# joe5saia/Hmc.jl

Measured on AMD Instinct MI355X. Metric: Gibbs draws/sec (whole node), 3-state T=1000 x256 windows per GPU, higher is better.
Workload: dtype f64

## Files before the change

hmc.jl_amd/csrc/gibbs_device.hpp:

```cpp
#pragma once
#include <hip/hip_runtime.h>
#include <stdint.h>

#include "../../include/hmcg.h"
#include "round5.hpp"

namespace hmcg {

enum { SITE_SIG2 = 0, SITE_MU = 1, SITE_RHO = 2, SITE_A = 3, SITE_X = 4, SITE_NOISE = 5 };
constexpr int GAMMA_MAX_ATTEMPTS = 64;
constexpr double INVSQRT2PI = 0.3989422804014327;
constexpr double TWO_PI = 6.283185307179586476925286766559;
constexpr double EPS64 = 2.220446049250313e-16;

struct KernelParams {
    const double* Y;
    const int32_t* T;
    const double* yreal;
    int32_t ldY, W, H;
    int32_t sweep_begin;
    int32_t sweep_end;
    int32_t resume;
    int32_t final_launch;
    int32_t horizons[HMCG_MAXH];
// ... 491 lines not shown
#pragma unroll
    for (int s = 0; s < K; ++s) {
        const uint32_t bs = (b >> (4 * s)) & 15u;
        m |= ((a >> (4u * bs)) & 15u) << (4 * s);
    }
    return m;
}
__device__ __forceinline__ int map_apply(uint32_t m, int s) { return (int)((m >> (4 * s)) & 15u); }

constexpr uint32_t BMAP_IDENTITY = 0x03020100u;
__device__ __forceinline__ uint32_t bmap_const(int v) { return (uint32_t)v * 0x01010101u; }
__device__ __forceinline__ uint32_t bmap_compose(uint32_t a, uint32_t b) { return __builtin_amdgcn_perm(a, a, b); }
__device__ __forceinline__ int bmap_apply(uint32_t m, int s) { return (int)((m >> (8 * s)) & 0xFFu); }
constexpr int DPP_ROW_SHL1 = 0x101, DPP_ROW_SHL2 = 0x102, DPP_ROW_SHL4 = 0x104, DPP_ROW_SHL8 = 0x108, DPP_WAVE_SHL1 = 0x130;

template <int K>
__device__ inline void matmul_small(double (&out)[K][K], const double (&a)[K][K], const double (&b)[K][K])
{
    double t[K][K];
#pragma unroll
    for (int i = 0; i < K; ++i)
#pragma unroll
        for (int j = 0; j < K; ++j) {
            double acc = 0.0;
#pragma unroll
            for (int k = 0; k < K; ++k) acc += a[i][k] * b[k][j];
            t[i][j] = acc;
        }
#pragma unroll
    for (int i = 0; i < K; ++i)
#pragma unroll
        for (int j = 0; j < K; ++j) out[i][j] = t[i][j];
}

template <int K>
__device__ inline double forecast_value(const double (&mu)[K], const double (&A)[K][K], const double (&pe)[K], int h)
{
    double M[K][K], v[K];
#pragma unroll
    for (int i = 0; i < K; ++i) {
        v[i] = mu[i];
#pragma unroll
        for (int j = 0; j < K; ++j) M[i][j] = A[i][j];
    }
    for (unsigned hh = (unsigned)h; hh != 0; hh >>= 1) {
        if (hh & 1u) {
            double nv[K];
#pragma unroll
            for (int i = 0; i < K; ++i) {
                double acc = 0.0;
#pragma unroll
                for (int j = 0; j < K; ++j) acc = fma(M[i][j], v[j], acc);
                nv[i] = acc;
            }
#pragma unroll
            for (int i = 0; i < K; ++i) v[i] = nv[i];
        }
        if (hh > 1u) matmul_small<K>(M, M, M);
    }
    double f = 0.0;
#pragma unroll
    for (int i = 0; i < K; ++i) f = fma(pe[i], v[i], f);
    return f;
}


template <int K>
struct ThetaBuf {
    double mu[K], sig2[K], isd[K], coef[K], rho[K];
    double A[K][K];
    double pi_end[K];
};

template <int K>
struct RngBuf {
    static constexpr int NG = K + K * K;
    double x[NG][2];
    double lu[NG][2];
    double uu[NG][2];
    double z[K];
    double rho[K];
};

template <int K, int L, int NT, bool SIG>
struct SweepShared {
    static constexpr int NW = NT / 64;
    static constexpr int NCNT = K + K * K;
    static constexpr int NF = K * K + (SIG ? K : 0);
    static constexpr int FW = (64 * L < 1024) ? 10 : 16;
    static constexpr int FPK = 32 / FW;
    static constexpr int NPK = (NF + FPK - 1) / FPK;
    unsigned red_pk[NW][NPK];
    double red_s1[SIG ? NW : 1][K];
    double red_s2[SIG ? NW : 1][K];
    int x_end;
    double red_d1[NW][K];
    double red_d2[NW][K];
    double pivot[K];
    ThetaBuf<K> th[2];
    RngBuf<K> rb[2];
    double wtot[NW][K * K];
    double pfirst[NT + 1][K];
    uint32_t wmap[NW];
    double ulast;
    int xfirst[NT + 1];
    double bred[NW];
    int selcnt[2][8][3];
    double ux[NT * L];
    double exptab[EXPTAB_N * EXPTAB_C];
    struct OutConst { double* base; double yr; int packed; int h; };
    OutConst oc[2][64];
    double ftail[2][SIG ? HMCG_MAXTAIL : 1][K];
    double pf_rep[2][K];
    double y_last[2];
};

template <int NW>
__device__ __forceinline__ double block_sum(double v, double* bred, int wave, int lane)
{
    v = wave_sum(v);
    __syncthreads();
    if (lane == 0 && wave < NW) bred[wave] = v;
    __syncthreads();
    double t = 0.0;
#pragma unroll
    for (int w = 0; w < NW; ++w) t += bred[w];
    return t;
}
template <int NW>
__device__ __forceinline__ double block_minmax(double v, double* bred, int wave, int lane, bool is_max)
{
    v = is_max ? wave_max(v) : wave_min(v);
    __syncthreads();
    if (lane == 0 && wave < NW) bred[wave] = v;
    __syncthreads();
    double t = bred[0];
#pragma unroll
    for (int w = 1; w < NW; ++w) t = is_max ? fmax(t, bred[w]) : fmin(t, bred[w]);
    return t;
}

__device__ __forceinline__ unsigned long long order_key(double v)
{
    const long long b = __double_as_longlong(v + 0.0);
    return (unsigned long long)(b ^ ((b >> 63) | (long long)0x8000000000000000ull));
}
__device__ __forceinline__ double key_value(unsigned long long k)
{
    return __longlong_as_double((long long)((k >> 63) ? (k ^ 0x8000000000000000ull) : ~k));
}
template <int NW, int NE, typename ElemFn>
__device__ __forceinline__ unsigned long long block_select(int n, ElemFn elem, int r, int (*cnt)[8][3], int wave, int lane)
{
    unsigned long long prefix = 0ull, mask = 0ull;
    const bool mine = __builtin_amdgcn_readfirstlane(wave) < NW;
    for (int b = 62; b >= 0; b -= 2) {
        const int par = (b >> 1) & 1;
        if (mine) {
            int c0 = 0, c1 = 0, c2 = 0;
            auto one = [&](int i) __attribute__((always_inline)) {
                unsigned long long key;
                const bool live = elem(i, key);
                const bool cand = live && ((key ^ prefix) & mask) == 0ull;
                const unsigned digit = (unsigned)(key >> b) & 3u;
                c0 += __builtin_popcountll(__builtin_amdgcn_ballot_w64(cand && digit == 0u));
                c1 += __builtin_popcountll(__builtin_amdgcn_ballot_w64(cand && digit == 1u));
                c2 += __builtin_popcountll(__builtin_amdgcn_ballot_w64(cand && digit == 2u));
            };
            if constexpr (NE > 0) {
#pragma unroll
                for (int i = 0; i < NE; ++i) one(i);
            } else {
                for (int i = 0; i < n; ++i) one(i);
            }
            if (lane == 0) { cnt[par][wave][0] = c0; cnt[par][wave][1] = c1; cnt[par][wave][2] = c2; }
        }
        __syncthreads();
        int t0 = 0, t1 = 0, t2 = 0;
#pragma unroll
        for (int w = 0; w < NW; ++w) { t0 += cnt[par][w][0]; t1 += cnt[par][w][1]; t2 += cnt[par][w][2]; }
        t0 = __builtin_amdgcn_readfirstlane(t0); t1 = __builtin_amdgcn_readfirstlane(t1); t2 = __builtin_amdgcn_readfirstlane(t2);
        unsigned long long digit = 0ull;
        if (r >= t0) { r -= t0; digit = 1ull;
            if (r >= t1) { r -= t1; digit = 2ull;
                if (r >= t2) { r -= t2; digit = 3ull; } } }
        prefix |= digit << b;
        mask |= 3ull << b;
    }
    return prefix;
}

template <int K>
__device__ __forceinline__ void sort_order(const double (&mu)[K], int (&order)[K])
{
    int pos[K];
#pragma unroll
    for (int i = 0; i < K; ++i) {
        int c = 0;
#pragma unroll
        for (int j = 0; j < K; ++j) c += (mu[j] < mu[i] || (mu[j] == mu[i] && j < i)) ? 1 : 0;
        pos[i] = c;
    }
#pragma unroll
    for (int q = 0; q < K; ++q) {
        int o = 0;
#pragma unroll
        for (int i = 0; i < K; ++i) o += (pos[i] == q) ? i : 0;
        order[q] = o;
    }
}

#ifdef HMCG_STAMPS
#define HMCG_NSTAMP 20
#define HMCG_NSTAMP_ALL (HMCG_NSTAMP + 2)
#define STAMP(i)                                                          \
    do {                                                                  \
        __builtin_amdgcn_sched_barrier(0);                                \
        asm volatile("; HMCG_STAMP_MARK %0" :: "n"(i));                    \
        const unsigned long long t_ = __builtin_amdgcn_s_memtime();       \
        __builtin_amdgcn_s_waitcnt(0xC07F);                               \
        __builtin_amdgcn_sched_barrier(0);                                \
        stamp_acc[i] += t_ - stamp_prev;                                  \
        stamp_prev = t_;                                                  \
    } while (0)
#else
#define STAMP(i)
#endif


template <int K, int L, int NT, bool SIG = false, bool SMOOTH = false, int NH = 0, int OCC = 1>
__global__ __launch_bounds__(NT + 64 * NH) __attribute__((amdgpu_waves_per_eu(OCC)))
void gibbs_sweeps_kernel(const KernelParams p)
{
    static_assert(NH == 0 || (NH == 4 && NT == 256), "helper waves: 256 + 256 threads");
    static_assert(K >= 2 && K <= 4, "small-K kernel: byte-per-entry state maps (v_perm_b32 composition)");
    static_assert(NT % 64 == 0 && NT >= 128, "at least two whole waves (wave 0 draws, the others work in its shadow)");
    constexpr int NW = NT / 64;
    constexpr int KK = K * K;
    constexpr int NG = K + KK;
    static_assert(NG <= 64, "draw roles must fit wave 0");
    using Sh = SweepShared<K, L, NT, SIG>;
    __shared__ Sh sh;

    int w_ = blockIdx.x;
    int t_lo_ = INT32_MIN, t_hi_ = INT32_MAX;
    if (p.order) {
        const int n_live = p.order[0];
        t_lo_ = p.order[1]; t_hi_ = p.order[2];
        if (n_live >= 0) {
            if (w_ >= n_live) __builtin_amdgcn_endpgm();
            w_ = p.order[4 + w_];
        }
    }
    const int w = w_;
#ifdef HMCG_VECTOR_WAVE
    const int tid = threadIdx.x, lane = tid & 63, wave = tid >> 6;
#else
    const int tid = threadIdx.x, lane = tid & 63, wave = __builtin_amdgcn_readfirstlane(tid >> 6);
#endif
    const int T = p.T[w];
    const int t0 = tid * L;
    const int owner = (T - 1) / L, l_last = (T - 1) % L;
    const bool helper = NH > 0 && __builtin_amdgcn_readfirstlane(wave) >= NW;
    int st = 0;

    if (T <= t_lo_ || T > t_hi_) __builtin_amdgcn_endpgm();
    if (T < 2 || T > NT * L || T > p.ldY) {
        if (tid == 0) flag_skipped(p, w, HMCG_ST_BAD_T);
        return;
    }

    exptab_fill(sh.exptab, tid, NT + 64 * NH);
    constexpr int XPAD = K < 4 ? K : 0;
    constexpr bool PADMARK = K < 4;
    double y[L];
    int x[L];
    bool bad = false;
#pragma unroll
    for (int l = 0; l < L; ++l) {
        const bool v = (t0 + l) < T;
        y[l] = v ? p.Y[(size_t)w * p.ldY + t0 + l] : 0.0;
        bad |= v && !isfinite(y[l]);
        x[l] = XPAD;
    }
    if (__syncthreads_or(bad ? 1 : 0)) {
        if (tid == 0) flag_skipped(p, w, HMCG_ST_NONFINITE);
        return;
    }
    int sb = T, se = T;
    double yreal[SIG ? L : 1];
    const double kfac = SIG ? 1.0 / (1.0 + p.kappa) : 1.0;
    if constexpr (SIG) {
        if (p.sig_range) { sb = p.sig_range[2 * w]; se = p.sig_range[2 * w + 1]; }
        bool bad_range = sb < 0 || se > T || (sb < se && se != T);
        if (p.save_range) {
            const int svb = p.save_range[2 * w], sve = p.save_range[2 * w + 1];
            bad_range |= svb < 0 || sve > T || (svb < sve && p.sigvals && sve - svb > p.nsave_ld);
        }
        if (bad_range) {
            if (tid == 0) flag_skipped(p, w, HMCG_ST_BAD_RANGE);
            return;
        }
        if (sb >= se) { sb = T; se = T; }
#pragma unroll
        for (int l = 0; l < L; ++l) yreal[l] = y[l];
    }
    int tail = 0;
    if constexpr (SIG) {
        if (p.end_pos) tail = (T - 1) - p.end_pos[w];
        if (tail < 0 || tail > HMCG_MAXTAIL || tail > T - 1) {
            if (tid == 0) flag_skipped(p, w, HMCG_ST_BAD_T);
            return;
        }
    }
    (void)kfac; (void)yreal; (void)sb; (void)se; (void)tail;

    double part = 0.0;
#pragma unroll
    for (int l = 0; l < L; ++l) part += y[l];
    const double xi = block_sum<NW>(part, sh.bred, wave, lane) / (double)T;

    double pivot[K];
#pragma unroll
    for (int k = 0; k < K; ++k) pivot[k] = xi;
// ... 234 lines not shown
            } else {
                double mu_u[K], pe_u[K], A_u[K][K];
#pragma unroll
                for (int i = 0; i < K; ++i) {
                    mu_u[i] = th.mu[i]; pe_u[i] = th.pi_end[i];
#pragma unroll
                    for (int j = 0; j < K; ++j) A_u[i][j] = th.A[i][j];
                }
                fv = forecast_value<K>(mu_u, A_u, pe_u, fc_h);
            }
            val = (o_which == 5) ? fv - fc_yr : fv;
        } else {
            double mu_u[K];
            int order[K];
#pragma unroll
            for (int i = 0; i < K; ++i) mu_u[i] = th.mu[i];
            sort_order<K>(mu_u, order);
            int si = 0, sj = 0;
#pragma unroll
            for (int qq = 0; qq < K; ++qq) {
                si = (qq == (o_which == 3 ? o_i : o_q)) ? order[qq] : si;
                sj = (qq == o_j) ? order[qq] : sj;
            }
            const double* src = o_which == 0 ? &th.mu[0] : (o_which == 1 ? &th.sig2[0] : (o_which == 2 ? &th.pi_end[0] : &th.A[0][0]));
            val = src[o_which == 3 ? si * K + sj : si];
            if constexpr (SIG) {
                if (tail > 0 && o_which == 2) {
                    double b[K];
#pragma unroll
                    for (int r = 0; r < K; ++r) b[r] = 1.0;
                    for (int j = tail - 1; j >= 0; --j) {
                        double g[K], nb[K];
#pragma unroll
                        for (int c = 0; c < K; ++c) g[c] = sh.ftail[sw & 1][j][c] * b[c];
#pragma unroll
                        for (int r = 0; r < K; ++r) {
                            double acc = 0.0;
#pragma unroll
                            for (int c = 0; c < K; ++c) acc = fma(th.A[r][c], g[c], acc);
                            nb[r] = acc;
                        }
                        rescale_pow2<K>(nb);
#pragma unroll
                        for (int r = 0; r < K; ++r) b[r] = nb[r];
                    }
                    double tot = 0.0, mine = 0.0;
#pragma unroll
                    for (int c = 0; c < K; ++c) {
                        const double g = sh.pf_rep[sw & 1][c] * b[c];
                        tot += g;
                        mine = (c == si) ? g : mine;
                    }
                    val = mine / tot;
                }
            }
        }
        if (out_base) ((__attribute__((address_space(1))) double*)out_base)[d - p.draw_off] = val;
        const double r5 = round5(val);
        sum_acc += r5;
        if constexpr (SIG) {
            if (p.sample_summary) {
                smp_acc += r5;
                const int smp = sw / p.per_sample;
                if (sw + 1 == (smp + 1) * p.per_sample) {
                    const int orole = (c.packed >> 20) & 63;
                    p.sample_summary[((size_t)w * p.n_samples + smp) * NS + orole] = p.nrun_s > 0 ? smp_acc / (double)p.nrun_s : __builtin_nan("");
                    smp_acc = 0.0;
                }
            }
        }
    };

#ifdef HMCG_STAMPS
    unsigned long long stamp_acc[HMCG_NSTAMP];
    unsigned long long stamp_prev = 0;
#endif
    constexpr int PB = L <= 1 ? 1 : (L <= 3 ? 2 : (L <= 7 ? 3 : (L <= 15 ? 4 : 5)));
    constexpr int FPW = 32 / PB;
    constexpr int NF = Sh::NF;
    constexpr int NWORD = (NF + FPW - 1) / FPW;
    constexpr int NPK = Sh::NPK;
    constexpr bool PADCNT = PADMARK && !SIG && NWORD == 1 && NF < FPW;
    static_assert(64 * L < 65536, "wave totals fit their fields (10 bits while 64 L < 1024, else 16)");
    auto publish_stats = [&]() __attribute__((always_inline)) {
        unsigned acc[NWORD];
#pragma unroll
        for (int wd = 0; wd < NWORD; ++wd) acc[wd] = 0;
#pragma unroll
        for (int l = 0; l < L; ++l) {
            const int xn = (l + 1 < L) ? x[(l + 1 < L) ? l + 1 : l] : xnext;
            const int code = PADCNT ? x[l] + K * xn : x[l] * K + xn;
            const bool pv = (t0 + l + 1) < T;
            if constexpr (PADCNT) {
                acc[0] += 1u << (PB * min(code, KK));
            } else if constexpr (NWORD == 1) {
                acc[0] += pv ? (1u << (PB * code)) : 0u;
            } else {
#pragma unroll
                for (int wd = 0; wd < NWORD; ++wd) {
                    const int rel = code - wd * FPW;
                    acc[wd] += (pv && rel >= 0 && rel < FPW) ? (1u << (PB * rel)) : 0u;
                }
            }
            if constexpr (SIG) {
                const int t = t0 + l;
                const bool sv = t >= sb && t < se;
                const int c2 = KK + x[l];
#pragma unroll
                for (int wd = 0; wd < NWORD; ++wd) {
                    const int rel = c2 - wd * FPW;
                    acc[wd] += (sv && rel >= 0 && rel < FPW) ? (1u << (PB * rel)) : 0u;
                }
            }
        }
        unsigned pk[NPK];
#pragma unroll
        for (int d = 0; d < NPK; ++d) {
            unsigned v = 0;
#pragma unroll
            for (int q = 0; q < Sh::FPK; ++q) {
                const int e = Sh::FPK * d + q;
                if (e < NF) v |= ((acc[e / FPW] >> (PB * (e % FPW))) & ((1u << PB) - 1u)) << (Sh::FW * q);
            }
            pk[d] = v;
        }
        wave_sum_words_lane63<NPK>(pk);
        double d1[K], d2[K], s1[SIG ? K : 1], s2[SIG ? K : 1];
#pragma unroll
        for (int i = 0; i < K; ++i) { d1[i] = 0.0; d2[i] = 0.0; }
        if constexpr (SIG) {
#pragma unroll
            for (int i = 0; i < K; ++i) { s1[i] = 0.0; s2[i] = 0.0; }
        }
#pragma unroll
        for (int l = 0; l < L; ++l) {
            double pvt = pivot[0];
#pragma unroll
            for (int k = 1; k < K; ++k) pvt = (x[l] == k) ? pivot[k] : pvt;
            const double dl = y[l] - pvt;
            const int t = t0 + l;
            const bool issig = SIG && t >= sb && t < se;
            const int xs = PADMARK ? (issig ? -1 : x[l]) : ((t < T && !issig) ? x[l] : -1);
#pragma unroll
            for (int i = 0; i < K; ++i) {
                const double dm = (xs == i) ? dl : 0.0;
                d1[i] += dm;
                d2[i] = fma(dm, dm, d2[i]);
            }
            if constexpr (SIG) {
                const int xg = issig ? x[l] : -1;
#pragma unroll
                for (int i = 0; i < K; ++i) {
                    const double dm = (xg == i) ? dl : 0.0;
                    s1[i] += dm;
                    s2[i] = fma(dm, dm, s2[i]);
                }
            }
        }
        if constexpr (SIG) {
            static_assert(!SIG || K <= 4, "signal path: transposed reduce carries 2 x 4 slots");
            double v8[8], o0, o1;
#pragma unroll
            for (int i = 0; i < 4; ++i) { v8[i] = i < K ? s1[i < K ? i : 0] : 0.0; v8[4 + i] = i < K ? s2[i < K ? i : 0] : 0.0; }
            wave_sum8_transposed(v8, lane, o0, o1);
            if ((lane & 0x3C) == 12) {
                const int i0 = lane & 2, i1 = i0 + 1;
                double* dst = (lane & 1) ? &sh.red_s2[wave][0] : &sh.red_s1[wave][0];
                if (i0 < K) dst[i0] = o0;
                if (i1 < K) dst[i1] = o1;
            }
        }
        if constexpr (K <= 4) {
            double v8[8], o0, o1;
#pragma unroll
            for (int i = 0; i < 4; ++i) { v8[i] = i < K ? d1[i] : 0.0; v8[4 + i] = i < K ? d2[i] : 0.0; }
            wave_sum8_transposed(v8, lane, o0, o1);
            if ((lane & 0x3C) == 12) {
                const int i0 = lane & 2, i1 = i0 + 1;
                double* dst = (lane & 1) ? &sh.red_d2[wave][0] : &sh.red_d1[wave][0];
                if (i0 < K) dst[i0] = o0;
                if (i1 < K) dst[i1] = o1;
            }
        } else {
#pragma unroll
            for (int i = 0; i < K; ++i) { d1[i] = wave_sum(d1[i]); d2[i] = wave_sum(d2[i]); }
            if (lane == 0) {
#pragma unroll
                for (int i = 0; i < K; ++i) { sh.red_d1[wave][i] = d1[i]; sh.red_d2[wave][i] = d2[i]; }
            }
        }
        if (lane == 63) {
#pragma unroll
            for (int d = 0; d < NPK; ++d) sh.red_pk[wave][d] = pk[d];
        }
        if (tid == 0) {
#pragma unroll
            for (int k = 0; k < K; ++k) sh.pivot[k] = pivot[k];
            sh.x_end = x_end;
        }
    };
    auto regen_y = [&](int smp, bool report) __attribute__((always_inline)) {
        if constexpr (SIG) {
            const double ssig = p.sigma_signal ? p.sigma_signal[w] : 0.0;
            const bool noisy = ssig != 0.0 || p.n_samples > 1;
            int svb = 0, sve = 0;
            if (p.save_range) { svb = p.save_range[2 * w]; sve = p.save_range[2 * w + 1]; }
            Rng gn = rng;
            gn.sweep = (uint32_t)smp;
#pragma unroll
            for (int l = 0; l < L; ++l) {
                const int t = t0 + l;
                if (noisy && t >= sb && t < se) {
                    uint32_t r[4];
                    gn.block(SITE_NOISE, 0, (uint32_t)t, r);
                    y[l] = yreal[l] + box_muller(r) * ssig;
                }
                if (report && p.sigvals && t >= svb && t < sve && t < T && (t - svb) < p.nsave_ld)
                    p.sigvals[((size_t)w * p.n_samples + smp) * p.nsave_ld + (t - svb)] = y[l];
                if (t == T - 1) sh.y_last[smp & 1] = y[l];
            }
        }
    };
    if constexpr (SIG) {
        if (p.sweep_begin % p.per_sample != 0) regen_y(p.sweep_begin / p.per_sample, false);
    }
    if (!helper) publish_stats();

    if (p.sweep_begin < p.sweep_end && shadow_wave == 0) job_prep(p.sweep_begin);

    uint32_t trips = 0;
    if constexpr (NH > 0) {
        const int ntrip = (((T + 1) >> 1) + 127) >> 7;
        constexpr int trip_wave[10] = {1, 2, 3, NW, 1, 2, 3, NW + 3, NW + 2, NW + 1};
        for (int k = 0; k < ntrip && k < 32; ++k) {
            const int wv = k < 10 ? trip_wave[k] : 1 + (k - 10) % 3;
            trips |= (wv == wave) ? (1u << k) : 0u;
        }
        trips = __builtin_amdgcn_readfirstlane(trips);
    }
    auto job_uniform_trips = [&](int sw) __attribute__((always_inline)) {
        const int nblk = (T + 1) >> 1;
        for (uint32_t m = trips; m != 0; m &= m - 1) {
            const int k = __builtin_ctz(m);
            job_uniforms(sw, k << 7, min((k << 7) + 128, nblk));
        }
    };

    double pf[L][K];
    double sm_acc[SMOOTH ? L : 1][K];
    double fm_acc[SMOOTH ? L : 1][K];
    if constexpr (SMOOTH) {
#pragma unroll
        for (int l = 0; l < L; ++l)
#pragma unroll
            for (int q = 0; q < K; ++q)
            {
                sm_acc[l][q] = (p.resume && p.pi_smooth_mean && t0 + l < T) ? p.pi_smooth_mean[((size_t)w * p.ldY + t0 + l) * K + q] : 0.0;
                fm_acc[l][q] = (p.resume && p.pi_filter_mean && t0 + l < T) ? p.pi_filter_mean[((size_t)w * p.ldY + t0 + l) * K + q] : 0.0;
            }
    }
    (void)sm_acc; (void)fm_acc;
#ifdef HMCG_STAMPS
    for (int i = 0; i < HMCG_NSTAMP; ++i) stamp_acc[i] = 0;
    stamp_prev = __builtin_amdgcn_s_memtime();
    const unsigned long long stamp_t0 = stamp_prev, stamp_r0 = __builtin_amdgcn_s_memrealtime();
#endif

    if constexpr (NH > 0) {
        if (helper) {
            for (int sweep = p.sweep_begin; sweep < p.sweep_end; ++sweep) {
                __syncthreads();
                STAMP(0);
                if (wave == PREP_WAVE && sweep + 1 < p.sweep_end) job_prep(sweep + 1);
                STAMP(15);
                job_uniform_trips(sweep);
                STAMP(1);
                __syncthreads();
                STAMP(2);
                if (sweep > p.sweep_begin) job_outputs(sweep - 1);
                STAMP(14);
                __syncthreads();
                __syncthreads();
                __syncthreads();
                STAMP(11);
            }
        }
    }

    for (int sweep = helper ? p.sweep_end : p.sweep_begin; sweep < p.sweep_end; ++sweep) {
        rng.sweep = (uint32_t)sweep;
        const int par = sweep & 1;
        ThetaBuf<K>& th = sh.th[par];
        if constexpr (SIG) {
            const int smp = sweep / p.per_sample;
            if (sweep == smp * p.per_sample) { regen_y(smp, true); publish_stats(); }
        }
        __syncthreads();
        STAMP(0);
        if (wave == 0) {
            const RngBuf<K>& rb = sh.rb[par];
            const int qi = (lane - 4) >> 2, qj = (lane - 4) & 3;
            const bool is_sig = lane < K, is_A = lane >= 4 && qi < K && qj < K;
            const bool is_g = is_sig || is_A;
            const int role = is_sig ? lane : (is_A ? K + qi * K + qj : NG);
            double shape = 1.0, bpar = 1.0, Neff = 0.0, Ssum = 0.0, rnn = 0.0;
            int cT = 0;
            {
                const int e = is_A ? (PADCNT ? qj * K + qi : role - K) : 0;
#pragma unroll
                for (int ww = 0; ww < NW; ++ww) cT += (int)((sh.red_pk[ww][e / Sh::FPK] >> (Sh::FW * (e % Sh::FPK))) & ((1u << Sh::FW) - 1u));
                cT = is_A ? cT : 0;
            }
            int rowsum = 0;
            {
                int qs = cT + __builtin_amdgcn_mov_dpp(cT, 0xB1, 0xF, 0xF, false);
                qs += __builtin_amdgcn_mov_dpp(qs, 0x4E, 0xF, 0xF, false);
#pragma unroll
                for (int i = 0; i < K; ++i) {
                    const int ri = __builtin_amdgcn_readlane(qs, 4 + 4 * i);
                    rowsum = (lane == i) ? ri : rowsum;
                }
            }
            STAMP(16);
            if (is_g) {
                const int c = is_sig ? rowsum + ((sh.x_end == role) ? 1 : 0) : cT;
                if (is_sig) {
                    double d1 = 0.0, d2 = 0.0;
#pragma unroll
                    for (int ww = 0; ww < NW; ++ww) { d1 += sh.red_d1[ww][role]; d2 += sh.red_d2[ww][role]; }
                    const double piv = sh.pivot[role];
                    const double beta = (sweep == 0) ? 1.0 : 2.0;
                    if constexpr (!SIG) {
                        Neff = (double)c;
                        const double rn = c > 0 ? rcp_fast(Neff) : 0.0;
                        const double ybar = c > 0 ? piv + d1 * rn : 0.0;
                        const double S2 = c > 0 ? fmax(d2 - d1 * d1 * rn, 0.0) : 0.0;
                        Ssum = piv * Neff + d1;
                        const double dm = ybar - xi;
                        shape = p.alpha + 0.5 * Neff;
                        rnn = rcp_fast(Neff + p.nu);
                        bpar = beta + 0.5 * S2 + 0.5 * Neff * p.nu * rnn * (dm * dm);
                    } else {
                        int Mi = 0;
                        {
                            const int e = KK + role;
#pragma unroll
                            for (int ww = 0; ww < NW; ++ww) Mi += (int)((sh.red_pk[ww][e / Sh::FPK] >> (Sh::FW * (e % Sh::FPK))) & ((1u << Sh::FW) - 1u));
                        }
                        const int Ni = c - Mi;
                        double g1 = 0.0, g2 = 0.0;
#pragma unroll
                        for (int ww = 0; ww < NW; ++ww) { g1 += sh.red_s1[ww][role]; g2 += sh.red_s2[ww][role]; }
                        const double dNi = (double)Ni, dMi = (double)Mi;
                        const double S = piv * dNi + d1, Sm = piv * dMi + g1;
                        const double S2 = Ni > 0 ? fmax(d2 - d1 * d1 / dNi, 0.0) : 0.0;
                        const double Sm2 = Mi > 0 ? fmax(g2 - g1 * g1 / dMi, 0.0) : 0.0;
                        const double totalbar = (Ni + Mi) > 0 ? (S + Sm) / (dNi + dMi) : 0.0;
                        Neff = dNi + dMi * kfac;
                        Ssum = S + Sm;
                        const double dm = totalbar - xi;
                        shape = p.alpha + 0.5 * dNi + 0.5 * dMi;
                        rnn = rcp_fast(Neff + p.nu);
                        bpar = beta + 0.5 * S2 + (0.5 * kfac) * Sm2 + 0.5 * Neff * p.nu * rnn * (dm * dm);
                    }
                } else {
                    shape = (double)(c + 1);
                }
            }
            STAMP(17);
            double val = 1.0;
            if (is_g) {
                const uint32_t site = role < K ? SITE_SIG2 : SITE_A;
                const uint32_t elem = role < K ? (uint32_t)role : (uint32_t)(role - K);
                if (shape == 1.0) {
                    uint32_t r[4];
                    rng.block(site, elem, 0, r);
                    val = -log_fast(1.0 - u53(r[0], r[1]));
                } else {
                    const double a = shape < 1.0 ? shape + 1.0 : shape;
                    const double dd = a - 1.0 / 3.0;
                    const double cc = rsqrt_fast(dd) * (1.0 / 3.0);
                    val = mt_try(dd, cc, rb.x[role][0], rb.lu[role][0], rb.uu[role][0]);
                    if (val < 0.0) val = mt_try(dd, cc, rb.x[role][1], rb.lu[role][1], rb.uu[role][1]);
                    if (val < 0.0) {
                        int j = 2;
                        for (; j < GAMMA_MAX_ATTEMPTS && val < 0.0; ++j) {
                            uint32_t r[4];
                            rng.block(site, elem, 2u * (uint32_t)j, r);
                            const double xx = box_muller(r);
                            rng.block(site, elem, 2u * (uint32_t)j + 1u, r);
                            const double u3 = u53(r[0], r[1]);
                            val = mt_try(dd, cc, xx, log_fast(1.0 - u3), u3);
                        }
                        if (val < 0.0) { val = dd; st |= HMCG_ST_GAMMA_CAP; }
                    }
                    if (shape < 1.0) {
                        uint32_t r[4];
                        rng.block(site, elem, 0xFFFFFFFFu, r);
                        val *= pow(1.0 - u53(r[0], r[1]), 1.0 / shape);
                    }
                }
            }
            STAMP(18);
            double gs = is_A ? val : 0.0;
            gs += quadperm_f64<0xB1>(gs);
            gs += quadperm_f64<0x4E>(gs);
            if (is_sig) {
                const double sig2 = bpar * rcp_fast(val);
                const double m = (Ssum + p.nu * xi) * rnn;
                const double sdev = sqrt_fast(sig2 * rnn);
                const double mu = m + sdev * rb.z[role];
                const double isd = rsqrt_fast(sig2);
                th.mu[role] = mu; th.sig2[role] = sig2;
                th.isd[role] = isd * 0.70710678118654752440; th.coef[role] = INVSQRT2PI * isd;
                th.rho[role] = rb.rho[role];
            } else if (is_A) {
                th.A[qi][qj] = val * rcp_fast(gs);
            }
        } else {
            const int nblk = (T + 1) >> 1;
            if (sweep > p.sweep_begin) job_outputs(sweep - 1);
            STAMP(14);
            if constexpr (NH > 0) {
                job_uniform_trips(sweep);
            } else if (NSH >= 3) {
                const int extra = NSH - 3;
                const int c_last = (nblk * 3) / 16;
                const int rest = nblk - c_last;
                const int den = 2 * (8 + 5) + 13 * extra;
                const int c0 = (rest * 16) / den, c1 = (rest * 10) / den;
                int b0, b1;
                if (shadow_wave == 0) { b0 = 0; b1 = c0; }
                else if (shadow_wave == 1) { b0 = c0; b1 = extra > 0 ? c0 + c1 : rest; }
                else if (shadow_wave == NSH - 1) { b0 = rest; b1 = nblk; }
                else {
                    const int per = extra > 0 ? (rest - c0 - c1 + extra - 1) / extra : 0;
                    b0 = c0 + c1 + (shadow_wave - 2) * per;
                    b1 = min(b0 + per, rest);
                }
                if (shadow_wave == 1 && sweep + 1 < p.sweep_end) job_prep(sweep + 1);
                STAMP(15);
                job_uniforms(sweep, b0, b1);
            } else {
                if (shadow_wave == 0 && sweep + 1 < p.sweep_end) job_prep(sweep + 1);
                const int per = (nblk + NSH - 1) / NSH;
                job_uniforms(sweep, shadow_wave * per, min((shadow_wave + 1) * per, nblk));
            }
        }
        STAMP(1);
        __syncthreads();
        STAMP(2);
        double mu[K], isd[K], coef[K], rho[K], A[K][K];
        int order[K];
#pragma unroll
        for (int i = 0; i < K; ++i) {
            mu[i] = th.mu[i]; isd[i] = th.isd[i]; coef[i] = th.coef[i]; rho[i] = th.rho[i];
#pragma unroll
            for (int j = 0; j < K; ++j) A[i][j] = th.A[i][j];
        }
        sort_order<K>(mu, order);
        double ux[L];
#pragma unroll
        for (int l = 0; l < L; ++l) ux[l] = sh.ux[t0 + l];
        double f[L][K];
        unsigned und = 0;
        if constexpr (L >= 8) {
#pragma unroll
            for (int l = 0; l < L; ++l) {
                unsigned hm = 0;
#pragma unroll
                for (int s = 0; s < K; ++s) {
                    double z = (y[l] - mu[s]) * isd[s];
                    double cf = coef[s];
                    if constexpr (SIG) {
                        const bool issig = (t0 + l) >= sb && (t0 + l) < se;
                        z = issig ? z * kfac : z;
                        cf = issig ? cf * kfac : cf;
                    }
                    f[l][s] = exp_tab(-(z * z), sh.exptab, lane & (EXPTAB_C - 1)) * cf;
                    hm = max(hm, (unsigned)__double2hiint(f[l][s]));
                }
                const int e = 1022 - (int)(hm >> 20);
#pragma unroll
                for (int s = 0; s < K; ++s) f[l][s] = ldexp(f[l][s], e);
                und |= (hm < 0x01A56E1Fu) ? (1u << l) : 0u;
            }
        } else {
            constexpr int LB = (16 / K) < L ? (16 / K) : L;
#define HMCG_EACH for (int g = 0; g < LB; ++g) _Pragma("unroll") for (int s = 0; s < K; ++s)
#define HMCG_SB __builtin_amdgcn_sched_barrier(0)
#pragma unroll
            for (int l0 = 0; l0 < L; l0 += LB) {
                double x[LB][K], nn[LB][K], tj[LB][K], r[LB][K], pp[LB][K];
                int ni[LB][K];
                auto LL = [&](int g) __attribute__((always_inline)) { return l0 + g < L ? l0 + g : L - 1; };
                auto issig = [&](int g) __attribute__((always_inline)) { return SIG && (t0 + LL(g)) >= sb && (t0 + LL(g)) < se; };
                HMCG_SB;
#pragma unroll
                HMCG_EACH x[g][s] = y[LL(g)] - mu[s];
                HMCG_SB;
#pragma unroll
                HMCG_EACH x[g][s] = x[g][s] * isd[s];
                if constexpr (SIG) {
                    HMCG_SB;
#pragma unroll
                    HMCG_EACH x[g][s] = issig(g) ? x[g][s] * kfac : x[g][s];
                }
                HMCG_SB;
#pragma unroll
                HMCG_EACH x[g][s] = -(x[g][s] * x[g][s]);
                HMCG_SB;
#pragma unroll
                HMCG_EACH x[g][s] = fmax(x[g][s], -746.0);
                HMCG_SB;
#pragma unroll
                HMCG_EACH nn[g][s] = x[g][s] * (EXPTAB_N == 64 ? 92.332482616893657 : 369.3299304675746);
                HMCG_SB;
#pragma unroll
                HMCG_EACH nn[g][s] = rint(nn[g][s]);
                HMCG_SB;
#pragma unroll
                HMCG_EACH ni[g][s] = (int)nn[g][s];
                HMCG_SB;
#pragma unroll
                HMCG_EACH tj[g][s] = exptab_at(sh.exptab, ni[g][s], lane & (EXPTAB_C - 1));
                HMCG_SB;
#pragma unroll
                HMCG_EACH r[g][s] = fma(-nn[g][s], EXPTAB_N == 64 ? 1.0830424693267560e-02 : 2.70760617331689e-03, x[g][s]);
                HMCG_SB;
#pragma unroll
                HMCG_EACH r[g][s] = fma(-nn[g][s], EXPTAB_N == 64 ? 2.9815858269852933e-12 : 7.453964567463233e-13, r[g][s]);
                HMCG_SB;
// ... 290 lines not shown
        STAMP(8);
        int xlast = 0;
        {
            const double ulast = sh.ulast;
            double cp = 0.0;
#pragma unroll
            for (int q = 0; q < K - 1; ++q) {
                double pq = 0.0;
#pragma unroll
                for (int s = 0; s < K; ++s) pq = (order[q] == s) ? th.pi_end[s] : pq;
                cp += pq;
                xlast += (cp <= ulast) ? 1 : 0;
            }
        }
        double pfn_last[K];
#pragma unroll
        for (int s = 0; s < K; ++s) pfn_last[s] = sh.pfirst[(tid + 1 < NT) ? tid + 1 : tid][s];
        uint32_t gmap[L];
        uint32_t G = BMAP_IDENTITY;
#pragma unroll
        for (int l = L - 1; l >= 0; --l) {
            const int t = t0 + l;
            uint32_t m = 0;
            int idx_uni = 0;
            {
                double ucum = 0.0;
#pragma unroll
                for (int r = 0; r < K - 1; ++r) { ucum += 1.0 / K; idx_uni += (ucum <= ux[l]) ? 1 : 0; }
            }
#pragma unroll
            for (int s = 0; s < K; ++s) {
                const double guard = (l + 1 < L) ? pf[(l + 1 < L) ? l + 1 : l][s] : pfn_last[s];
                double tot = 0.0;
                int idx = 0;
                double cum[K];
#pragma unroll
                for (int r = 0; r < K; ++r) { tot = fma(pf[l][r], A[r][s], tot); cum[r] = tot; }
                const double thr = ux[l] * tot;
#pragma unroll
                for (int r = 0; r < K - 1; ++r) idx += (cum[r] <= thr) ? 1 : 0;
                idx = (guard > EPS64) ? idx : idx_uni;
                m |= (uint32_t)idx << (8 * s);
            }
            if constexpr (K < 4) m |= BMAP_IDENTITY & (0xFFFFFFFFu << (8 * K));
            m = (t == T - 1) ? bmap_const(xlast) : (t > T - 1 ? (PADMARK ? bmap_const(XPAD) : BMAP_IDENTITY) : m);
            gmap[l] = m;
            G = bmap_compose(m, G);
        }
        STAMP(9);
        uint32_t Hm = G;
        Hm = bmap_compose(Hm, (uint32_t)dpp_i32<DPP_ROW_SHL1, 0xF>((int)BMAP_IDENTITY, (int)Hm));
        Hm = bmap_compose(Hm, (uint32_t)dpp_i32<DPP_ROW_SHL2, 0xF>((int)BMAP_IDENTITY, (int)Hm));
        Hm = bmap_compose(Hm, (uint32_t)dpp_i32<DPP_ROW_SHL4, 0xF>((int)BMAP_IDENTITY, (int)Hm));
        Hm = bmap_compose(Hm, (uint32_t)dpp_i32<DPP_ROW_SHL8, 0xF>((int)BMAP_IDENTITY, (int)Hm));
        {
            const uint32_t R1 = (uint32_t)__builtin_amdgcn_readlane((int)Hm, 16);
            const uint32_t R2 = (uint32_t)__builtin_amdgcn_readlane((int)Hm, 32);
            const uint32_t R3 = (uint32_t)__builtin_amdgcn_readlane((int)Hm, 48);
            const uint32_t S1 = bmap_compose(R2, R3), S0 = bmap_compose(R1, S1);
            const int row = lane >> 4;
            const uint32_t after = row == 0 ? S0 : (row == 1 ? S1 : (row == 2 ? R3 : BMAP_IDENTITY));
            Hm = bmap_compose(Hm, after);
        }
        if (lane == 0) sh.wmap[wave] = Hm;
        STAMP(10);
        __syncthreads();
        STAMP(11);
        uint32_t Rw = BMAP_IDENTITY;
#pragma unroll
        for (int ww = NW - 1; ww >= 1; --ww) if (ww > wave_u) Rw = bmap_compose(sh.wmap[ww], Rw);
        const uint32_t Hx = (uint32_t)dpp_i32<DPP_WAVE_SHL1, 0xF>((int)BMAP_IDENTITY, (int)Hm);
        const uint32_t Sfx = bmap_compose(Hx, Rw);
        int sin = bmap_apply(Sfx, XPAD);
        xnext = sin;
        x_end = xlast;
#pragma unroll
        for (int l = L - 1; l >= 0; --l) {
            sin = bmap_apply(gmap[l], sin);
            x[l] = sin;
        }
#pragma unroll
        for (int k = 0; k < K; ++k) pivot[k] = mu[k];
        STAMP(12);
        publish_stats();
        STAMP(13);
    }
#ifdef HMCG_STAMPS
    if (lane == 0 && p.dbg) {
        unsigned long long* o = p.dbg + ((size_t)w * (NW + NH) + wave) * HMCG_NSTAMP_ALL;
        for (int i = 0; i < HMCG_NSTAMP; ++i) o[i] = stamp_acc[i];
        o[HMCG_NSTAMP] = __builtin_amdgcn_s_memtime() - stamp_t0;
        o[HMCG_NSTAMP + 1] = __builtin_amdgcn_s_memrealtime() - stamp_r0;
    }
#endif

    __syncthreads();
    if (p.sweep_end > p.sweep_begin) job_outputs(p.sweep_end - 1);
    if (p.xstate) {
#pragma unroll
        for (int l = 0; l < L; ++l) if (t0 + l < T) p.xstate[(size_t)w * p.ldY + t0 + l] = (uint8_t)x[l];
    }
    if (p.x_final) {
#pragma unroll
        for (int l = 0; l < L; ++l) if (t0 + l < T) p.x_final[(size_t)w * p.ldY + t0 + l] = x[l];
    }
    if (p.pif_final && p.sweep_end > p.sweep_begin) {
#pragma unroll
        for (int l = 0; l < L; ++l)
            if (t0 + l < T)
#pragma unroll
                for (int s = 0; s < K; ++s) p.pif_final[((size_t)w * p.ldY + t0 + l) * K + s] = pf[l][s];
    }
    if constexpr (SMOOTH) {
        if (p.pi_filter_mean) {
            const double sc = (p.final_launch && p.nd > 0) ? 1.0 / (double)p.nd : 1.0;
#pragma unroll
            for (int l = 0; l < L; ++l)
                if (t0 + l < T)
#pragma unroll
                    for (int q = 0; q < K; ++q) p.pi_filter_mean[((size_t)w * p.ldY + t0 + l) * K + q] = fm_acc[l][q] * sc;
        }
        if (p.pi_smooth_mean) {
            const double sc = (p.final_launch && p.nd > 0) ? 1.0 / (double)p.nd : 1.0;
#pragma unroll
            for (int l = 0; l < L; ++l)
                if (t0 + l < T)
#pragma unroll
                    for (int q = 0; q < K; ++q) p.pi_smooth_mean[((size_t)w * p.ldY + t0 + l) * K + q] = sm_acc[l][q] * sc;
        }
    }
    {
        const int orole = role_of(lane);
        if (orole >= 0) {
            if (p.sumacc) p.sumacc[(size_t)w * NCK + orole] = sum_acc;
            if (p.summary && p.final_launch)
                p.summary[(size_t)w * NS + orole] = p.nd > 0 ? sum_acc / (double)p.nd : __builtin_nan("");
            if constexpr (SIG) {
                if (p.sample_summary) {
                    const int smp = p.sweep_end / p.per_sample, kb = p.sweep_end - smp * p.per_sample - p.burnin_s;
                    if (kb > 0 && kb < p.nrun_s && smp < p.n_samples) p.sample_summary[((size_t)w * p.n_samples + smp) * NS + orole] = smp_acc;
                }
            }
        }
    }
    if (p.sumacc) {
#pragma unroll
        for (int k = 0; k < K; ++k) if (tid == k) p.sumacc[(size_t)w * NCK + (NCK - K) + k] = pivot[k];
    }
    if (st) atomicOr(&p.status[w], st);
}

}
```

hmc.jl_amd/csrc/hmcg.hip:

```cpp
#include <hip/hip_runtime.h>

#include <algorithm>
#include <chrono>
#include <cstdarg>
#include <cstdlib>
#include <cstdio>
#include <cstring>
#include <condition_variable>
#include <functional>
#include <mutex>
#include <numeric>
#include <string>
#include <thread>
#include <vector>

#include "host_util.hpp"
#include "moments.hpp"
#include "variants.hpp"

namespace {

thread_local char g_err[512] = "";

void set_err(const char* fmt, ...)
// ... 403 lines not shown
{
    const size_t stride = (size_t)W + ORD_HDR;
    int32_t* meta = ord + (size_t)MAXBUCKET * stride;
    const int w = (int)(blockIdx.x * blockDim.x + threadIdx.x);
    if (w < W) {
        auto bucket_of = [&](int t) { int k = 0; for (int b = 0; b < r.nb; ++b) if (t > r.lo[b] && t <= r.hi[b]) k = b; return k; };
        const int mine = bucket_of(T[w]);
        int32_t* list = ord + (size_t)mine * stride;
        const int pos = atomicAdd(&list[0], 1);
        list[ORD_HDR + pos] = w;
        if (w > 0 && bucket_of(T[w - 1]) != mine) atomicAdd(&meta[0], 1);
    }
    __threadfence();
    __syncthreads();
    if (threadIdx.x == 0 && atomicAdd(&meta[1], 1) == (int)gridDim.x - 1) {
        __threadfence();
        int runs = 0;
        for (int b = 0; b < r.nb; ++b) runs += atomicAdd(&ord[(size_t)b * stride], 0) > 0 ? 1 : 0;
        const bool sorted = atomicAdd(&meta[0], 0) == runs - 1 || !r.compact;
        for (int b = 0; b < r.nb; ++b) {
            int32_t* list = ord + (size_t)b * stride;
            if (sorted) list[0] = -1;
            list[1] = r.lo[b]; list[2] = r.hi[b];
        }
    }
}
size_t bucket_list_bytes(int W) { return sizeof(int32_t) * ((size_t)MAXBUCKET * ((size_t)W + ORD_HDR) + 2); }
int build_bucket_lists(const Plan& pl, const int32_t* dT, int W, int32_t* ord, hipStream_t stream)
{
    BucketRanges r{};
    r.nb = pl.nb;
    r.compact = diag_env("HMCG_NO_BUCKET_LISTS") ? 0 : 1;
    for (int b = 0; b < pl.nb; ++b) { r.lo[b] = pl.b[b].t_lo; r.hi[b] = pl.b[b].t_hi; }
    HIP_TRY(hipMemsetAsync(ord, 0, bucket_list_bytes(W), stream));
    hipLaunchKernelGGL(bucket_lists_kernel, dim3((unsigned)((W + 255) / 256)), dim3(256), 0, stream, dT, W, r, ord);
    HIP_TRY(hipGetLastError());
    return 0;
}

int launch_kernel(DeviceCtx& c, const Plan& pl, const hmcg::KernelParams& p, hipStream_t stream, const int32_t* ord)
{
    if (pl.nb > 1) {
        HIP_TRY(hipEventRecord(c.ev_fork, stream));
        for (int b = 0; b < pl.nb; ++b) {
            hipStream_t bs = b == 0 ? stream : c.bstream[b - 1];
            if (b > 0) HIP_TRY(hipStreamWaitEvent(bs, c.ev_fork, 0));
            hmcg::KernelParams q = p;
            q.order = ord + (size_t)b * ((size_t)p.W + ORD_HDR);
            const Variant* v = pl.b[b].v;
            hipLaunchKernelGGL(v->fn, dim3((unsigned)p.W), dim3((unsigned)(v->NT + 64 * v->NH)), 0, bs, q);
            HIP_TRY(hipGetLastError());
            if (b > 0) HIP_TRY(hipEventRecord(c.ev_join[b - 1], bs));
        }
        for (int b = 1; b < pl.nb; ++b) HIP_TRY(hipStreamWaitEvent(stream, c.ev_join[b - 1], 0));
        return 0;
    }
    if (pl.v) hipLaunchKernelGGL(pl.v->fn, dim3((unsigned)p.W), dim3((unsigned)(pl.v->NT + 64 * pl.v->NH)), 0, stream, p);
    else hipLaunchKernelGGL(pl.bv->fn, dim3((unsigned)p.W), dim3((unsigned)pl.bv->NT), pl.dyn, stream, p, pl.bigL);
    HIP_TRY(hipGetLastError());
    return 0;
}

void fill_timing(hmcg_timing* t, const Plan& pl, const DeviceCtx& c, double kernel_ms, int launches, double call_ms, int windows)
{
    if (!t) return;
    t->kernel_ms = kernel_ms;
    t->launches = launches;
    t->threads_per_window = pl.NT();
    t->steps_per_thread = pl.L();
    t->helper_waves = pl.NH();
    t->device = c.device;
    t->call_ms = call_ms;
    t->windows = windows;
    t->occupancy = pl.v ? pl.v->occ : 0;
    t->buckets = pl.nb > 1 ? pl.nb : 1;
    t->streaming = pl.stream ? 1 : 0;
    t->lds_bytes = (int32_t)(static_lds_bytes(pl.fptr(), 0) + pl.dyn);
}

#ifdef HMCG_STAMPS
int print_stamps(const hmcg::KernelParams& p, const Plan& pl, unsigned long long* ddbg, size_t ndbg, hipStream_t stream)
{
    static const char* names[HMCG_NSTAMP] = {"Ba wait", "param draws | shadow jobs", "Bb wait", "theta+ux+pdfs", "local product",
        "wave scan", "Bc wait", "prefix+replay+last", "Bd wait", "maps+compose", "map scan", "Be wait", "apply", "publish stats", "  (shadow: outputs)", "  (shadow: prep)", "  (param: counts+row sums)", "  (param: shapes)", "  (param: gamma)", "unused"};
    const int nwv = pl.NT() / 64 + pl.NH();
    std::vector<unsigned long long> h(ndbg);
    HIP_TRY(hipStreamSynchronize(stream));
    static int launches_seen = 0;
    static const int print_after = diag_env("HMCG_STAMPS_AFTER") ? atoi(diag_env("HMCG_STAMPS_AFTER")) : 0;
    if (launches_seen++ < print_after) return 0;
    HIP_TRY(hipMemcpy(h.data(), ddbg, ndbg * sizeof(unsigned long long), hipMemcpyDeviceToHost));
    const int nsw = p.sweep_end - p.sweep_begin;
    {
        std::vector<double> clk;
        double ticks = 0;
        for (int w = 0; w < p.W; ++w)
            for (int wv = 0; wv < nwv; ++wv) {
                const unsigned long long* o = &h[((size_t)w * nwv + wv) * HMCG_NSTAMP_ALL];
                if (o[HMCG_NSTAMP + 1]) { clk.push_back(100.0 * (double)o[HMCG_NSTAMP] / (double)o[HMCG_NSTAMP + 1]); ticks += (double)o[HMCG_NSTAMP]; }
            }
        std::sort(clk.begin(), clk.end());
        if (!clk.empty())
            fprintf(stderr, "[clock] launch %d: in-kernel clock MHz min %.0f median %.0f max %.0f (s_memtime / s_memrealtime x 100 MHz); "
                            "%.0f ticks per sweep (mean over waves)\n", launches_seen - 1, clk.front(), clk[clk.size() / 2], clk.back(),
                    ticks / (double)clk.size() / (nsw > 0 ? nsw : 1));
    }
    fprintf(stderr, "[stamps] K=%d L=%d NT=%d W=%d sweeps=%d: mean cycles per sweep by wave (s_memtime ticks)\n",
            pl.v ? pl.v->K : pl.bv->K, pl.L(), pl.NT(), p.W, nsw);
    fprintf(stderr, "%-24s", "phase");
    for (int wv = 0; wv < nwv; ++wv) fprintf(stderr, "   wave%-2d", wv);
    fprintf(stderr, "\n");
    std::vector<double> tot(nwv, 0.0);
    for (int i = 0; i < HMCG_NSTAMP; ++i) {
        fprintf(stderr, "%-24s", names[i]);
        for (int wv = 0; wv < nwv; ++wv) {
            double acc = 0;
            for (int w = 0; w < p.W; ++w) acc += (double)h[((size_t)w * nwv + wv) * HMCG_NSTAMP_ALL + i];
            acc /= (double)p.W * (nsw > 0 ? nsw : 1);
            tot[wv] += acc;
            fprintf(stderr, " %8.0f", acc);
        }
        fprintf(stderr, "\n");
    }
    fprintf(stderr, "%-24s", "total");
    for (int wv = 0; wv < nwv; ++wv) fprintf(stderr, " %8.0f", tot[wv]);
    fprintf(stderr, "\n");
    return 0;
}
#endif

int launch_device(DeviceCtx& c, const hmcg_config* cfg, const double* dY, const int32_t* dT, const double* dyreal, double* dmu,
                  double* dsig2, double* dA, double* dpi_end, double* dfcast, double* dsummary, int32_t* dstatus,
                  const hmcg_extras* ex, hipStream_t stream, hmcg_timing* timing)
{
    if (!dY || !dT || !dstatus) { set_err("Y, T and status are required"); return HMCG_E_BADARG; }
    Plan pl;
    int rc = make_plan(cfg, ex, cfg->W, c.cu_count, cfg->min_T, nullptr, &pl);
    if (rc) return rc;
    if (pl.needs_pif() && !(ex && ex->pif_final)) {
        set_err("pi_smooth_mean / pi_filter_mean for K >= 5 or windows beyond the register-resident kernels need extras.pif_final "
                "([W][ldY][K]: the running sweep's filtered probabilities pass through it)");
        return HMCG_E_BADARG;
    }
    if (ex && ex->corr && (!dmu || !dsig2 || !dA || !dpi_end || !dfcast)) {
        set_err("extras.corr on the device entry needs all five per-draw outputs");
        return HMCG_E_BADARG;
    }
    const bool resume = (cfg->flags & HMCG_FLAG_RESUME) != 0;
    hmcg::KernelParams p = base_params(cfg, cfg->W, dY, dT, dyreal, dstatus, ex, pl.use_sig);
    const int total_sweeps = p.n_samples * (cfg->burnin + cfg->nrun);
    p.sweep_begin = cfg->sweep_base;
    p.sweep_end = total_sweeps;
    if (cfg->sweep_count > 0 && cfg->sweep_base + cfg->sweep_count < p.sweep_end) p.sweep_end = cfg->sweep_base + cfg->sweep_count;
    p.resume = resume ? 1 : 0;
    p.final_launch = (p.sweep_end == total_sweeps) ? 1 : 0;
    p.mu = dmu; p.sig2 = dsig2; p.A = dA; p.pi_end = dpi_end; p.fcast = dfcast; p.summary = dsummary;
    p.nd_ld = p.nd; p.draw_off = 0;

    if (!resume) HIP_TRY(hipMemsetAsync(dstatus, 0, sizeof(int32_t) * (size_t)cfg->W, stream));
    const bool use_lists = pl.nb > 1;
    const bool uses_scratch = pl.bv != nullptr || (ex && ex->corr) || use_lists;
    if (uses_scratch) HIP_TRY(hipStreamWaitEvent(stream, c.ev_scr, 0));
    int32_t* ord = nullptr;
    if (use_lists) {
        if (c.ord.cap < bucket_list_bytes(cfg->W)) HIP_TRY(hipStreamSynchronize(stream));
        if (c.ord.ensure(bucket_list_bytes(cfg->W))) { set_err("workspace allocation failed (%zu B device)", bucket_list_bytes(cfg->W)); return HMCG_E_NOMEM; }
        ord = reinterpret_cast<int32_t*>(c.ord.base);
// ... 560 lines not shown
```

Baseline: 54.10 million.

## Offload per-state residual sums to helper waves via packed LDS state buffer

When helper waves are present and SIG is off, main waves now publish only transition counts plus byte-packed states to a new LDS buffer. The helper waves read those states, the pivots and their own reloaded Y values, then compute the per-state d1/d2 residual sums at the start of the next sweep, overlapping with parameter draws. The sigma/mu draw is split around an extra block barrier so it can consume the helper-computed sums. This shortens the main waves' critical path at the cost of extra barriers, extra LDS, and a Y copy held in helper registers.

```diff
diff --git a/hmc.jl_amd/csrc/gibbs_device.hpp b/hmc.jl_amd/csrc/gibbs_device.hpp
--- a/hmc.jl_amd/csrc/gibbs_device.hpp
+++ b/hmc.jl_amd/csrc/gibbs_device.hpp
@@ -597,7 +597,7 @@
     double rho[K];
 };
 
-template <int K, int L, int NT, bool SIG>
+template <int K, int L, int NT, bool SIG, int XW = 0>
 struct SweepShared {
     static constexpr int NW = NT / 64;
     static constexpr int NCNT = K + K * K;
@@ -628,6 +628,7 @@
     double ftail[2][SIG ? HMCG_MAXTAIL : 1][K];
     double pf_rep[2][K];
     double y_last[2];
+    unsigned xb[XW > 0 ? XW : 1][XW > 0 ? NT : 1];
 };
 
 template <int NW>
@@ -726,7 +727,7 @@
 }
 
 #ifdef HMCG_STAMPS
-#define HMCG_NSTAMP 20
+#define HMCG_NSTAMP 23
 #define HMCG_NSTAMP_ALL (HMCG_NSTAMP + 2)
 #define STAMP(i)                                                          \
     do {                                                                  \
@@ -754,7 +755,9 @@
     constexpr int KK = K * K;
     constexpr int NG = K + KK;
     static_assert(NG <= 64, "draw roles must fit wave 0");
-    using Sh = SweepShared<K, L, NT, SIG>;
+    constexpr bool SPLIT = NH > 0 && !SIG;
+    constexpr int XW = (L + 3) / 4;
+    using Sh = SweepShared<K, L, NT, SIG, SPLIT ? XW : 0>;
     __shared__ Sh sh;
 
     int w_ = blockIdx.x;
@@ -1155,7 +1158,7 @@
     constexpr int NPK = Sh::NPK;
     constexpr bool PADCNT = PADMARK && !SIG && NWORD == 1 && NF < FPW;
     static_assert(64 * L < 65536, "wave totals fit their fields (10 bits while 64 L < 1024, else 16)");
-    auto publish_stats = [&]() __attribute__((always_inline)) {
+    auto count_words = [&](unsigned (&pk)[NPK]) __attribute__((always_inline)) {
         unsigned acc[NWORD];
 #pragma unroll
         for (int wd = 0; wd < NWORD; ++wd) acc[wd] = 0;
@@ -1186,7 +1189,6 @@
                 }
             }
         }
-        unsigned pk[NPK];
 #pragma unroll
         for (int d = 0; d < NPK; ++d) {
             unsigned v = 0;
@@ -1198,6 +1200,19 @@
             pk[d] = v;
         }
         wave_sum_words_lane63<NPK>(pk);
+    };
+    auto store_counts = [&](const unsigned (&pk)[NPK]) __attribute__((always_inline)) {
+        if (lane == 63) {
+#pragma unroll
+            for (int d = 0; d < NPK; ++d) sh.red_pk[wave][d] = pk[d];
+        }
+        if (tid == 0) {
+#pragma unroll
+            for (int k = 0; k < K; ++k) sh.pivot[k] = pivot[k];
+            sh.x_end = x_end;
+        }
+    };
+    auto publish_sums = [&](const int (&xv)[L], const double (&pv)[K], int tv, int wv) __attribute__((always_inline)) {
         double d1[K], d2[K], s1[SIG ? K : 1], s2[SIG ? K : 1];
 #pragma unroll
         for (int i = 0; i < K; ++i) { d1[i] = 0.0; d2[i] = 0.0; }
@@ -1207,13 +1222,13 @@
         }
 #pragma unroll
         for (int l = 0; l < L; ++l) {
-            double pvt = pivot[0];
-#pragma unroll
-            for (int k = 1; k < K; ++k) pvt = (x[l] == k) ? pivot[k] : pvt;
+            double pvt = pv[0];
+#pragma unroll
+            for (int k = 1; k < K; ++k) pvt = (xv[l] == k) ? pv[k] : pvt;
             const double dl = y[l] - pvt;
-            const int t = t0 + l;
+            const int t = tv + l;
             const bool issig = SIG && t >= sb && t < se;
-            const int xs = PADMARK ? (issig ? -1 : x[l]) : ((t < T && !issig) ? x[l] : -1);
+            const int xs = PADMARK ? (issig ? -1 : xv[l]) : ((t < T && !issig) ? xv[l] : -1);
 #pragma unroll
             for (int i = 0; i < K; ++i) {
                 const double dm = (xs == i) ? dl : 0.0;
@@ -1221,7 +1236,7 @@
                 d2[i] = fma(dm, dm, d2[i]);
             }
             if constexpr (SIG) {
-                const int xg = issig ? x[l] : -1;
+                const int xg = issig ? xv[l] : -1;
 #pragma unroll
                 for (int i = 0; i < K; ++i) {
                     const double dm = (xg == i) ? dl : 0.0;
@@ -1238,7 +1253,7 @@
             wave_sum8_transposed(v8, lane, o0, o1);
             if ((lane & 0x3C) == 12) {
                 const int i0 = lane & 2, i1 = i0 + 1;
-                double* dst = (lane & 1) ? &sh.red_s2[wave][0] : &sh.red_s1[wave][0];
+                double* dst = (lane & 1) ? &sh.red_s2[wv][0] : &sh.red_s1[wv][0];
                 if (i0 < K) dst[i0] = o0;
                 if (i1 < K) dst[i1] = o1;
             }
@@ -1250,7 +1265,7 @@
             wave_sum8_transposed(v8, lane, o0, o1);
             if ((lane & 0x3C) == 12) {
                 const int i0 = lane & 2, i1 = i0 + 1;
-                double* dst = (lane & 1) ? &sh.red_d2[wave][0] : &sh.red_d1[wave][0];
+                double* dst = (lane & 1) ? &sh.red_d2[wv][0] : &sh.red_d1[wv][0];
                 if (i0 < K) dst[i0] = o0;
                 if (i1 < K) dst[i1] = o1;
             }
@@ -1259,17 +1274,31 @@
             for (int i = 0; i < K; ++i) { d1[i] = wave_sum(d1[i]); d2[i] = wave_sum(d2[i]); }
             if (lane == 0) {
 #pragma unroll
-                for (int i = 0; i < K; ++i) { sh.red_d1[wave][i] = d1[i]; sh.red_d2[wave][i] = d2[i]; }
-            }
-        }
-        if (lane == 63) {
-#pragma unroll
-            for (int d = 0; d < NPK; ++d) sh.red_pk[wave][d] = pk[d];
-        }
-        if (tid == 0) {
-#pragma unroll
-            for (int k = 0; k < K; ++k) sh.pivot[k] = pivot[k];
-            sh.x_end = x_end;
+                for (int i = 0; i < K; ++i) { sh.red_d1[wv][i] = d1[i]; sh.red_d2[wv][i] = d2[i]; }
+            }
+        }
+    };
+    auto publish_stats = [&]() __attribute__((always_inline)) {
+        unsigned pk[NPK];
+        count_words(pk);
+        publish_sums(x, pivot, t0, wave);
+        store_counts(pk);
+    };
+    auto publish_counts = [&]() __attribute__((always_inline)) {
+        unsigned pk[NPK];
+        count_words(pk);
+        store_counts(pk);
+    };
+    auto publish_states = [&]() __attribute__((always_inline)) {
+        if constexpr (SPLIT) {
+#pragma unroll
+            for (int q = 0; q < XW; ++q) {
+                unsigned v = 0;
+#pragma unroll
+                for (int r = 0; r < 4; ++r)
+                    if (4 * q + r < L) v |= ((unsigned)x[4 * q + r < L ? 4 * q + r : 0] & 0xFFu) << (8 * r);
+                sh.xb[q][tid] = v;
+            }
         }
     };
     auto regen_y = [&](int smp, bool report) __attribute__((always_inline)) {
@@ -1298,6 +1327,13 @@
         if (p.sweep_begin % p.per_sample != 0) regen_y(p.sweep_begin / p.per_sample, false);
     }
     if (!helper) publish_stats();
+    if constexpr (SPLIT) {
+        if (helper) {
+            const int tm = (tid - NT) * L;
+#pragma unroll
+            for (int l = 0; l < L; ++l) y[l] = (tm + l) < T ? p.Y[(size_t)w * p.ldY + tm + l] : 0.0;
+        }
+    }
 
     if (p.sweep_begin < p.sweep_end && shadow_wave == 0) job_prep(p.sweep_begin);
 
@@ -1305,8 +1341,9 @@
     if constexpr (NH > 0) {
         const int ntrip = (((T + 1) >> 1) + 127) >> 7;
         constexpr int trip_wave[10] = {1, 2, 3, NW, 1, 2, 3, NW + 3, NW + 2, NW + 1};
+        constexpr int trip_wave_split[10] = {1, 2, 3, 1, 2, 3, NW + 1, NW + 2, NW + 3, NW};
         for (int k = 0; k < ntrip && k < 32; ++k) {
-            const int wv = k < 10 ? trip_wave[k] : 1 + (k - 10) % 3;
+            const int wv = k < 10 ? (SPLIT ? trip_wave_split[k] : trip_wave[k]) : 1 + (k - 10) % 3;
             trips |= (wv == wave) ? (1u << k) : 0u;
         }
         trips = __builtin_amdgcn_readfirstlane(trips);
@@ -1344,12 +1381,33 @@
             for (int sweep = p.sweep_begin; sweep < p.sweep_end; ++sweep) {
                 __syncthreads();
                 STAMP(0);
-                if (wave == PREP_WAVE && sweep + 1 < p.sweep_end) job_prep(sweep + 1);
-                STAMP(15);
+                if constexpr (SPLIT) {
+                    if (sweep > p.sweep_begin) {
+                        int xh[L];
+#pragma unroll
+                        for (int l = 0; l < L; ++l) xh[l] = (int)((sh.xb[l >> 2][tid - NT] >> (8 * (l & 3))) & 0xFFu);
+                        double ph[K];
+#pragma unroll
+                        for (int k = 0; k < K; ++k) ph[k] = sh.pivot[k];
+                        publish_sums(xh, ph, (tid - NT) * L, wave - NW);
+                    }
+                    STAMP(20);
+                } else {
+                    if (wave == PREP_WAVE && sweep + 1 < p.sweep_end) job_prep(sweep + 1);
+                    STAMP(15);
+                }
                 job_uniform_trips(sweep);
                 STAMP(1);
+                if constexpr (SPLIT) {
+                    __syncthreads();
+                    STAMP(21);
+                }
                 __syncthreads();
                 STAMP(2);
+                if constexpr (SPLIT) {
+                    if (wave == PREP_WAVE && sweep + 1 < p.sweep_end) job_prep(sweep + 1);
+                    STAMP(15);
+                }
                 if (sweep > p.sweep_begin) job_outputs(sweep - 1);
                 STAMP(14);
                 __syncthreads();
@@ -1377,6 +1435,8 @@
             const bool is_g = is_sig || is_A;
             const int role = is_sig ? lane : (is_A ? K + qi * K + qj : NG);
             double shape = 1.0, bpar = 1.0, Neff = 0.0, Ssum = 0.0, rnn = 0.0;
+            int c_sig = 0;
+            double rn_sig = 0.0, nn_sig = 0.0;
             int cT = 0;
             {
                 const int e = is_A ? (PADCNT ? qj * K + qi : role - K) : 0;
@@ -1397,7 +1457,14 @@
             STAMP(16);
             if (is_g) {
                 const int c = is_sig ? rowsum + ((sh.x_end == role) ? 1 : 0) : cT;
-                if (is_sig) {
+                if (SPLIT && is_sig) {
+                    Neff = (double)c;
+                    const double rn = c > 0 ? rcp_fast(Neff) : 0.0;
+                    shape = p.alpha + 0.5 * Neff;
+                    rnn = rcp_fast(Neff + p.nu);
+                    c_sig = c; rn_sig = rn;
+                    nn_sig = 0.5 * Neff * p.nu * rnn;
+                } else if (is_sig) {
                     double d1 = 0.0, d2 = 0.0;
 #pragma unroll
                     for (int ww = 0; ww < NW; ++ww) { d1 += sh.red_d1[ww][role]; d2 += sh.red_d2[ww][role]; }
@@ -1478,7 +1545,37 @@
             double gs = is_A ? val : 0.0;
             gs += quadperm_f64<0xB1>(gs);
             gs += quadperm_f64<0x4E>(gs);
-            if (is_sig) {
+            if constexpr (SPLIT) {
+                if (is_A) th.A[qi][qj] = val * rcp_fast(gs);
+                const double rval = rcp_fast(val);
+                const double piv = sh.pivot[role < K ? role : 0];
+                const double zr = rb.z[role < K ? role : 0];
+                if (is_sig) th.rho[role] = rb.rho[role];
+                STAMP(1);
+                __syncthreads();
+                STAMP(21);
+                if (is_sig) {
+                    const int c = c_sig;
+                    const double rn = rn_sig;
+                    double d1 = 0.0, d2 = 0.0;
+#pragma unroll
+                    for (int ww = 0; ww < NW; ++ww) { d1 += sh.red_d1[ww][role]; d2 += sh.red_d2[ww][role]; }
+                    const double beta = (sweep == 0) ? 1.0 : 2.0;
+                    const double ybar = c > 0 ? piv + d1 * rn : 0.0;
+                    const double S2 = c > 0 ? fmax(d2 - d1 * d1 * rn, 0.0) : 0.0;
+                    Ssum = piv * Neff + d1;
+                    const double dm = ybar - xi;
+                    bpar = beta + 0.5 * S2 + nn_sig * (dm * dm);
+                    const double sig2 = bpar * rval;
+                    const double m = (Ssum + p.nu * xi) * rnn;
+                    const double sdev = sqrt_fast(sig2 * rnn);
+                    const double mu = m + sdev * zr;
+                    const double isd = rsqrt_fast(sig2);
+                    th.mu[role] = mu; th.sig2[role] = sig2;
+                    th.isd[role] = isd * 0.70710678118654752440; th.coef[role] = INVSQRT2PI * isd;
+                }
+                STAMP(22);
+            } else if (is_sig) {
                 const double sig2 = bpar * rcp_fast(val);
                 const double m = (Ssum + p.nu * xi) * rnn;
                 const double sdev = sqrt_fast(sig2 * rnn);
@@ -1496,6 +1593,11 @@
             STAMP(14);
             if constexpr (NH > 0) {
                 job_uniform_trips(sweep);
+                if constexpr (SPLIT) {
+                    STAMP(1);
+                    __syncthreads();
+                    STAMP(21);
+                }
             } else if (NSH >= 3) {
                 const int extra = NSH - 3;
                 const int c_last = (nblk * 3) / 16;
@@ -1520,7 +1622,7 @@
                 job_uniforms(sweep, shadow_wave * per, min((shadow_wave + 1) * per, nblk));
             }
         }
-        STAMP(1);
+        if constexpr (!SPLIT) { STAMP(1); }
         __syncthreads();
         STAMP(2);
         double mu[K], isd[K], coef[K], rho[K], A[K][K];
@@ -1977,8 +2079,15 @@
 #pragma unroll
         for (int k = 0; k < K; ++k) pivot[k] = mu[k];
         STAMP(12);
-        publish_stats();
-        STAMP(13);
+        if constexpr (SPLIT) {
+            publish_counts();
+            STAMP(13);
+            publish_states();
+            STAMP(19);
+        } else {
+            publish_stats();
+            STAMP(13);
+        }
     }
 #ifdef HMCG_STAMPS
     if (lane == 0 && p.dbg) {
diff --git a/hmc.jl_amd/csrc/hmcg.hip b/hmc.jl_amd/csrc/hmcg.hip
--- a/hmc.jl_amd/csrc/hmcg.hip
+++ b/hmc.jl_amd/csrc/hmcg.hip
@@ -509,7 +509,8 @@
 int print_stamps(const hmcg::KernelParams& p, const Plan& pl, unsigned long long* ddbg, size_t ndbg, hipStream_t stream)
 {
     static const char* names[HMCG_NSTAMP] = {"Ba wait", "param draws | shadow jobs", "Bb wait", "theta+ux+pdfs", "local product",
-        "wave scan", "Bc wait", "prefix+replay+last", "Bd wait", "maps+compose", "map scan", "Be wait", "apply", "publish stats", "  (shadow: outputs)", "  (shadow: prep)", "  (param: counts+row sums)", "  (param: shapes)", "  (param: gamma)", "unused"};
+        "wave scan", "Bc wait", "prefix+replay+last", "Bd wait", "maps+compose", "map scan", "Be wait", "apply", "publish stats", "  (shadow: outputs)", "  (shadow: prep)", "  (param: counts+row sums)", "  (param: shapes)", "  (param: gamma)", "x store",
+        "  (helper: sums)", "Bx wait", "  (param: after Bx)"};
     const int nwv = pl.NT() / 64 + pl.NH();
     std::vector<unsigned long long> h(ndbg);
     HIP_TRY(hipStreamSynchronize(stream));
```

After: 54.76 million, median of 6. 1.01x the previous value.
